# leotimus/recommender-tensorflow

Hardware: AMD Instinct MI355X
Metric: examples/sec DeepFM batch=65536 (full train step) (higher is better)
Workload: dtype f32 (MLP GEMM operands: fp16 hi+lo split, 3 products, fp32 accumulate)

## Files before the change

recommender-tensorflow_amd/csrc/gemm_pl.hip:

```cpp
#include "common.h"
#include "planes.h"
#include <algorithm>
#include <cstdlib>
#include <type_traits>

namespace {

typedef _Float16 f16x8 __attribute__((ext_vector_type(8)));
typedef float f32x16 __attribute__((ext_vector_type(16)));

constexpr int PL_THREADS = 512;
constexpr int PL_BK = 16;

enum { PL_FWD = 0, PL_DGRAD = 1, PL_TOP = 2 };

struct PlArgs {
  const char* A; int64_t bsa; const int32_t* a_exp;
  const char* B; int64_t bsb; const int32_t* b_exp;
  int M, N, K;
  int tiles_n;
  float* C; int64_t ldc;
  char* Cp; int64_t bsc; int32_t* c_exp;
  const float* bias; int relu; float keep_prob, keep_div, keep_rcp; uint64_t seed;
  const char* mask; int64_t bsm;
  uint32_t* mbits; int64_t mbld;
  float* amax_c;
  const mi_step_state_t* st;
  const float* top_w; const float* top_b;
  const float* top_lin; const float* top_lin_bias; const float* top_fm; const uint8_t* top_labels; float top_scale;
  float* top_dnn; float* top_logits; float* top_dlogit;
  float* top_part;
};

#ifdef MI_PL_STAMPS
__device__ long long g_pl_stamps[32 * 2 * 128 * 8];
#define PL_STAMP(slot) do { if (stamp_on && t < 128) g_pl_stamps[((stamp_wg * 2 + stamp_grp) * 128 + t) * 8 + (slot)] = clock64(); } while (0)
#define PL_MARK(row) do { if (stamp_on) g_pl_stamps[((stamp_wg * 2 + stamp_grp) * 128 + (row)) * 8 + 7] = clock64(); } while (0)
#else
#define PL_STAMP(slot) do {} while (0)
#define PL_MARK(row) do {} while (0)
#endif

template <int TN, int TM, int EPI, bool HOT = false>
__global__ __launch_bounds__(PL_THREADS, 2) void gemm_pl_k(const PlArgs a) {
  constexpr int PL_NBUF = TN == 1 ? 3 : 4;
  constexpr int BNt = 128 * TN, BMt = 64 * TM, ROWS = BNt + BMt;
  constexpr int LPS = ROWS * 4 / PL_THREADS;
  static_assert(ROWS * 4 % PL_THREADS == 0, "tile rows");
  constexpr int STAGE = ROWS * PL_ROWB;
  static_assert(PL_NBUF * STAGE <= 160 * 1024, "LDS");
  __shared__ __attribute__((aligned(1024))) char smem[PL_NBUF * STAGE];

  const int nb = gridDim.x, bid = blockIdx.x;
  const int qq = nb >> 3, rr = nb & 7, xcd = bid & 7, idx = bid >> 3;
  const int lid = (xcd < rr) ? xcd * (qq + 1) + idx : rr * (qq + 1) + (xcd - rr) * qq + idx;
  const int n0 = (lid % a.tiles_n) * BNt, m0 = (lid / a.tiles_n) * BMt;
  const int nk = a.K / PL_BK;

  const int t = threadIdx.x, lane = t & 63;
  const int wv = __builtin_amdgcn_readfirstlane(t >> 6);
  const int i = lane & 31, h = lane >> 5;
  const int wn = wv & 3, wm = wv >> 2;

  const char* src[LPS];
#pragma unroll
  for (int j = 0; j < LPS; ++j) {
    const int p = j * PL_THREADS + t;
    const int row = p >> 2, c = (p & 3) ^ ((row >> 2) & 3);
    if (j < TN) {
      const int n = min(n0 + row, a.N - 1);
      src[j] = a.A + static_cast<int64_t>(n) * PL_ROWB + c * 16;
    } else {
      const int m = min(m0 + row - BNt, a.M - 1);
      src[j] = a.B + static_cast<int64_t>(m) * PL_ROWB + c * 16;
    }
  }

  const int sw = (i >> 2) & 3;
  const int ch = (h ^ sw) * 16, cl = ((2 | h) ^ sw) * 16;
  const int offA = (wn * 32 * TN + i) * PL_ROWB;
  const int offB = (BNt + wm * 32 * TM + i) * PL_ROWB;

  f32x16 acc[TN][TM];
#pragma unroll
  for (int x = 0; x < TN; ++x)
#pragma unroll
    for (int y = 0; y < TM; ++y)
#pragma unroll
      for (int r = 0; r < 16; ++r) acc[x][y][r] = 0.f;

  auto issue_share = [&](int kt, int buf) {
#pragma unroll
    for (int j = 0; j < LPS; ++j)
      __builtin_amdgcn_global_load_lds((const __attribute__((address_space(1))) void*)(src[j] + kt * (j < TN ? a.bsa : a.bsb)),
                                       (__attribute__((address_space(3))) void*)(smem + buf * STAGE + (j * PL_THREADS + wv * 64) * 16),
                                       16, 0, 0);
  };
  f16x8 ah[TN], al[TN], bh[TM], bl[TM];
  auto read_frags = [&](int bufi) {
    const char* buf = smem + bufi * STAGE;
#pragma unroll
    for (int x = 0; x < TN; ++x) {
      ah[x] = *reinterpret_cast<const f16x8*>(buf + offA + x * 32 * PL_ROWB + ch);
      al[x] = *reinterpret_cast<const f16x8*>(buf + offA + x * 32 * PL_ROWB + cl);
    }
#pragma unroll
    for (int y = 0; y < TM; ++y) {
      bh[y] = *reinterpret_cast<const f16x8*>(buf + offB + y * 32 * PL_ROWB + ch);
      bl[y] = *reinterpret_cast<const f16x8*>(buf + offB + y * 32 * PL_ROWB + cl);
    }
  };
  constexpr bool DMA_IN_C = TN != 1;
  auto phase_c = [&](int t) {
    int fb = t - 1 + PL_NBUF;
    fb -= (fb / PL_NBUF) * PL_NBUF;
    const int kt = min(t - 1 + PL_NBUF, nk - 1);
    constexpr int NT = TN * TM, NM = 3 * NT, GAP = NM / (LPS + 1);
#pragma unroll
    for (int idx = 0; idx < NM; ++idx) {
      const int pr = idx / NT, x = (idx % NT) / TM, y = idx % TM;
      acc[x][y] = __builtin_amdgcn_mfma_f32_32x32x16_f16(pr == 0 ? al[x] : ah[x], pr == 1 ? bl[y] : bh[y], acc[x][y], 0, 0, 0);
      if (DMA_IN_C && (idx + 1) % GAP == 0 && (idx + 1) / GAP <= LPS) {
        const int j = (idx + 1) / GAP - 1;
        __builtin_amdgcn_sched_barrier(0);
        __builtin_amdgcn_global_load_lds((const __attribute__((address_space(1))) void*)(src[j] + kt * (j < TN ? a.bsa : a.bsb)),
                                         (__attribute__((address_space(3))) void*)(smem + fb * STAGE + (j * PL_THREADS + wv * 64) * 16),
                                         16, 0, 0);
        __builtin_amdgcn_sched_barrier(0);
      }
    }
  };
  auto phase_l = [&](int t) {
    if (!DMA_IN_C && t >= 1) {
      int fb = t - 1;
      fb -= (fb / PL_NBUF) * PL_NBUF;
      issue_share(min(t - 1 + PL_NBUF, nk - 1), fb);
    }
    int rb = t;
    rb -= (rb / PL_NBUF) * PL_NBUF;
    read_frags(rb);
  };
  const bool g1 = __builtin_amdgcn_readfirstlane(wm) != 0;

#ifdef MI_PL_STAMPS
  const int stamp_every = max(1, nb / 32);
  const bool stamp_on = lane == 0 && (wv == 0 || wv == 4) && lid % stamp_every == 0 && lid / stamp_every < 32;
  const int stamp_wg = lid / stamp_every, stamp_grp = wv >> 2;
#endif
  PL_MARK(0);
#pragma unroll
  for (int s = 0; s < PL_NBUF; ++s) issue_share(min(s, nk - 1), s);
  mi_wait_vmcnt<LPS*(PL_NBUF - 1)>();
  __builtin_amdgcn_s_barrier();
  if (g1) __builtin_amdgcn_s_barrier();
  PL_MARK(1);
#pragma unroll 1
  for (int t = 0; t < nk; ++t) {
    PL_STAMP(0);
    phase_l(t);
    PL_STAMP(1);
    asm volatile("s_waitcnt lgkmcnt(0)" ::: "memory");
    PL_STAMP(2);
    mi_wait_vmcnt<LPS*(DMA_IN_C ? PL_NBUF - 3 : PL_NBUF - 2)>();
    PL_STAMP(3);
    __builtin_amdgcn_sched_barrier(0);
    __builtin_amdgcn_s_barrier();
    __builtin_amdgcn_sched_barrier(0);
    PL_STAMP(4);
    __builtin_amdgcn_s_setprio(1);
    phase_c(t);
    __builtin_amdgcn_s_setprio(0);
    PL_STAMP(5);
    __builtin_amdgcn_sched_barrier(0);
    __builtin_amdgcn_s_barrier();
    __builtin_amdgcn_sched_barrier(0);
    PL_STAMP(6);
  }
  if (!g1) __builtin_amdgcn_s_barrier();
  PL_MARK(2);

  if constexpr (EPI == PL_TOP) {
    static_assert(TN == 1, "PL_TOP: one 128-column tile");
    mi_wait_vmcnt<0>();
    __syncthreads();
    float* e_fw = reinterpret_cast<float*>(smem);
    float* e_bias = e_fw + 128;
    float* e_w = e_bias + 128;
    float* e_part = e_w + 128;
    float* e_dw = e_part + 4 * BMt;
    float* e_sc = e_dw + 256;
    float* e_wmax = e_sc + 4;
    static_assert((128 * 3 + 4 * BMt + 256 + 4 + 8) * 4 <= 8192 && 8192 + 8 * 4096 <= PL_NBUF * STAGE, "PL_TOP LDS");
    char* wreg = smem + 8192 + wv * 4096;
    for (int n = t; n < 128; n += PL_THREADS) {
      const bool ok = n < a.N;
      e_fw[n] = ok ? pl_pow2(-a.a_exp[ok ? n : 0]) : 0.f;
      e_bias[n] = (a.bias && ok) ? a.bias[n] : 0.f;
      e_w[n] = ok ? a.top_w[n] : 0.f;
    }
    __syncthreads();
    const bool drop = a.keep_prob < 1.f;
    const uint32_t thresh16 = drop ? mi_drop_thresh16(a.keep_prob) : 0x10000u;
    const uint64_t seed = a.seed + (a.st ? a.st->seed_term : 0ull);
    const int nw = wn * 32;
    const uint32_t pair_base = static_cast<uint32_t>((nw + 4 * h) >> 1) * MI_DROP_PAIR_MUL;
    const float kd = a.keep_div, kr = a.keep_rcp;
    const float relu_floor = a.relu ? 0.f : -__builtin_inff();
    float wr[16];
#pragma unroll
    for (int g = 0; g < 4; ++g) {
// ... 133 lines not shown
      for (int q = 0; q < 4; ++q) {
        auto r1 = __builtin_amdgcn_permlane32_swap(ph[q], ph[q + 4], false, false);
        ph[q] = r1[0]; ph[q + 4] = r1[1];
        auto r2 = __builtin_amdgcn_permlane32_swap(pq[q], pq[q + 4], false, false);
        pq[q] = r2[0]; pq[q + 4] = r2[1];
      }
      char* d = wreg + (h * 32 + i) * 64;
      const int rot = (i >> 1) & 3;
      *reinterpret_cast<uint4*>(d + ((0 ^ rot) << 4)) = make_uint4(ph[0], ph[1], ph[4], ph[5]);
      *reinterpret_cast<uint4*>(d + ((1 ^ rot) << 4)) = make_uint4(ph[2], ph[3], ph[6], ph[7]);
      *reinterpret_cast<uint4*>(d + ((2 ^ rot) << 4)) = make_uint4(pq[0], pq[1], pq[4], pq[5]);
      *reinterpret_cast<uint4*>(d + ((3 ^ rot) << 4)) = make_uint4(pq[2], pq[3], pq[6], pq[7]);
      asm volatile("s_waitcnt lgkmcnt(0)" ::: "memory");
#pragma unroll
      for (int q = 0; q < 4; ++q) {
        const int off = q * 1024 + lane * 16;
        const int blk = off >> 11, row = (off >> 6) & 31, slot = (off >> 4) & 3;
        const uint4 v4 = *reinterpret_cast<const uint4*>(wreg + off);
        const int mm = m0 + wm * 32 * TM + y * 32 + row, ncol = nw + blk * 16;
        if (mm < a.M && ncol < a.N)
          *reinterpret_cast<uint4*>(a.Cp + (ncol >> 4) * a.bsc + static_cast<int64_t>(mm) * PL_ROWB + ((slot ^ ((row >> 1) & 3)) << 4)) = v4;
      }
      asm volatile("s_waitcnt lgkmcnt(0)" ::: "memory");
    }
    return;
  }

  mi_wait_vmcnt<0>();
  __syncthreads();
  float* e_fw = reinterpret_cast<float*>(smem);
  float* e_bias = e_fw + BNt;
  float* e_rmax = e_bias + BNt;
  float* e_wmax = e_rmax + 4 * BMt;
  constexpr int FS = TN * 128 + 16;
  constexpr int WREG = 32 * FS > TN * 4096 ? 32 * FS : TN * 4096;
  constexpr int WPR = BNt / 32;
  static_assert(8192 + 8 * WREG + BMt * WPR * 4 <= PL_NBUF * STAGE, "epilogue LDS");
  char* wreg = smem + 8192 + wv * WREG;
  uint32_t* e_bits = reinterpret_cast<uint32_t*>(smem + 8192 + 8 * WREG);
  for (int n = t; n < BNt; n += PL_THREADS) {
    const int gn = n0 + n;
    const bool ok = HOT || gn < a.N;
    e_fw[n] = ok ? pl_pow2(-a.a_exp[ok ? gn : 0]) : 0.f;
    e_bias[n] = (EPI == PL_FWD && a.bias && ok) ? a.bias[gn] : 0.f;
  }
  __syncthreads();

  const bool drop = EPI == PL_FWD && (HOT || a.keep_prob < 1.f);
  float* const Cf = HOT ? nullptr : a.C;
  const uint32_t thresh16 = drop ? mi_drop_thresh16(a.keep_prob) : 0x10000u;
  const uint64_t seed = a.seed + (a.st ? a.st->seed_term : 0ull);
  const int nw = wn * 32 * TN;
  const uint32_t pair_base = static_cast<uint32_t>((n0 + nw + 4 * h) >> 1) * MI_DROP_PAIR_MUL;
  const bool bitmask = EPI == PL_DGRAD && (HOT || a.mbits != nullptr);
  const bool masked = !HOT && EPI == PL_DGRAD && a.mask != nullptr && !bitmask;
  const bool divide = drop || masked || bitmask;
  const float kd = divide ? a.keep_div : 1.f, kr = divide ? a.keep_rcp : 1.f;
  const float relu_floor = a.relu ? 0.f : -__builtin_inff();
  float rmx[TM];
#pragma unroll
  for (int y = 0; y < TM; ++y) {
    const int m = m0 + wm * 32 * TM + y * 32 + i;
    const bool mok = HOT || m < a.M;
    const int mc = mok ? m : a.M - 1;
    const float fx = pl_pow2(-a.b_exp[mc]);
    float mx = 0.f;
    const uint32_t rowkey = drop ? mi_drop_rowkey(seed, static_cast<uint32_t>(m)) : 0u;
    auto col_of = [&](int gi) { return nw + (gi >> 2) * 32 + 8 * (gi & 3) + 4 * h; };
    float4 fw_n = *reinterpret_cast<const float4*>(e_fw + col_of(0));
    float4 b_n = make_float4(0.f, 0.f, 0.f, 0.f);
// ... 470 lines not shown
}

__global__ __launch_bounds__(256) void top_fold_k(const float* __restrict__ part, int nparts, int N, float* __restrict__ dW,
                                                  float* __restrict__ db, float* __restrict__ d_sum, float* __restrict__ loss) {
  __shared__ float red[16][17];
  const int c = threadIdx.x & 15, sl = threadIdx.x >> 4;
  const int k = blockIdx.x * 16 + c;
  float acc = 0.f;
  if (k < N + 2) {
#pragma unroll 8
    for (int q = sl; q < nparts; q += 16) acc += part[static_cast<int64_t>(q) * (N + 2) + k];
  }
  red[sl][c] = acc;
  __syncthreads();
  if (sl == 0 && k < N + 2) {
    float v = 0.f;
#pragma unroll
    for (int q = 0; q < 16; ++q) v += red[q][c];
    if (k < N) dW[k] = v;
    else if (k == N) { if (db) db[0] = v; if (d_sum) d_sum[0] = v; }
    else if (loss) loss[0] = v;
  }
}

template <int EPI>
int32_t launch_pl(PlArgs& a, hipStream_t st, const char* what) {
  int tn = a.N <= 128 ? 1 : (a.N <= 256 ? 2 : 4);
  if (a.N > 512) tn = 2;
  if (const int v = mi::env_int("MI_PL_TILE", 0)) {
    if ((v == 1 || v == 2 || v == 4) && (!a.Cp || a.N <= 128 * v)) tn = v;
  }
  int tm = tn == 4 ? 2 : 4;
  if (tm == 4 && static_cast<int64_t>((a.N + 128 * tn - 1) / (128 * tn)) * ((a.M + 255) / 256) < 256) tm = 2;
  const int bn = 128 * tn, bm = 64 * tm;
  a.tiles_n = (a.N + bn - 1) / bn;
  const int64_t blocks = static_cast<int64_t>(a.tiles_n) * ((a.M + bm - 1) / bm);
  if (blocks <= 0 || blocks > INT32_MAX) {
    mi::set_error("%s: bad grid", what);
    return MI_ERR_INVALID;
  }
  if (a.Cp && a.tiles_n != 1) {
    mi::set_error("%s: a planes result needs N <= 512 (one column tile holds the whole row)", what);
    return MI_ERR_UNSUPPORTED;
  }
  const dim3 g(static_cast<unsigned>(blocks)), b(PL_THREADS);
  const bool hot = a.Cp && !a.C && a.tiles_n == 1 && a.N == bn && a.M % bm == 0 && a.amax_c && a.bsc < (int64_t(1) << 31) &&
                   (EPI == PL_FWD ? (a.keep_prob < 1.f && a.mbits && a.mbld * 32 == a.N && a.bias)
                                  : (a.mbits && a.mbld * 32 == a.N));
  if (hot && tn == 1 && tm == 4) gemm_pl_k<1, 4, EPI, true><<<g, b, 0, st>>>(a);
  else if (hot && tn == 2 && tm == 4) gemm_pl_k<2, 4, EPI, true><<<g, b, 0, st>>>(a);
  else if (hot && tn == 4 && EPI == PL_DGRAD) gemm_pl_k<4, 2, PL_DGRAD, true><<<g, b, 0, st>>>(a);
  else if (tn == 1 && tm == 4) gemm_pl_k<1, 4, EPI><<<g, b, 0, st>>>(a);
  else if (tn == 1) gemm_pl_k<1, 2, EPI><<<g, b, 0, st>>>(a);
  else if (tn == 2 && tm == 4) gemm_pl_k<2, 4, EPI><<<g, b, 0, st>>>(a);
  else if (tn == 2) gemm_pl_k<2, 2, EPI><<<g, b, 0, st>>>(a);
  else gemm_pl_k<4, 2, EPI><<<g, b, 0, st>>>(a);
  MI_CHECK_LAUNCH(what);
  return MI_OK;
}

}

extern "C" {

size_t mi_planes_bytes(int64_t rows, int32_t K) { return static_cast<size_t>((K + 15) >> 4) * static_cast<size_t>(rows) * PL_ROWB; }

int32_t mi_split_rows(const float* X, int64_t ldx, int64_t rows, int32_t K, int32_t transpose, const mi_planes_t* out,
                      float* amax_out, mi_stream_t stream) {
  MI_REQUIRE(rows >= 0 && K > 0 && X, "split_rows: rows=%lld K=%d", (long long)rows, K);
  if (rows == 0) return MI_OK;
  MI_REQUIRE(mi::planes_ok(out, rows), "split_rows: output planes (16-byte aligned data, blk_stride >= 64 * rows and a multiple of 64, row_exp)");
  MI_REQUIRE(transpose ? ldx >= rows : ldx >= K, "split_rows: ldx=%lld", (long long)ldx);
  if (transpose) {
    const int64_t tb = mi::ceil_div(rows, 32);
    MI_REQUIRE(tb <= INT32_MAX, "split_rows: grid too large");
    split_t_k<<<dim3((unsigned)tb), dim3(256), 0, mi::as_stream(stream)>>>(X, ldx, rows, K, static_cast<char*>(out->data),
                                                                           out->blk_stride, out->row_exp, amax_out);
    MI_CHECK_LAUNCH("split_rows(transposed)");
    return MI_OK;
  }
  if ((K & 15) == 0 && (ldx & 3) == 0 && (reinterpret_cast<uintptr_t>(X) & 15u) == 0) {
    int lpr = 1;
    while (lpr < 64 && lpr < (K >> 4)) lpr <<= 1;
// ... 57 lines not shown
  MI_CHECK_LAUNCH("merge_rows");
  return MI_OK;
}

int32_t mi_dense_fwd_planes(const mi_planes_t* X, const mi_planes_t* Wt, const float* bias, float* Y, int64_t ldy,
                            const mi_planes_t* Yp, int64_t M, int32_t N, int32_t K, int32_t relu, float keep_prob,
                            uint64_t seed, float* amax_out, uint32_t* mask_bits_out, int64_t mask_ld, mi_stream_t stream) {
  MI_REQUIRE(M >= 0 && M <= INT32_MAX && N > 0 && K > 0, "dense_fwd_planes: M=%lld N=%d K=%d", (long long)M, N, K);
  MI_REQUIRE(!mask_bits_out || mask_ld >= (N + 31) / 32, "dense_fwd_planes: mask_ld=%lld < ceil(N / 32)", (long long)mask_ld);
  if (M == 0) return MI_OK;
  MI_REQUIRE((K & 15) == 0 && (N & 15) == 0, "dense_fwd_planes: N=%d and K=%d must be multiples of 16 (use mi_dense_fwd)", N, K);
  MI_REQUIRE(mi::planes_ok(X, M) && mi::planes_ok(Wt, N), "dense_fwd_planes: operand planes");
  MI_REQUIRE(Y || Yp, "dense_fwd_planes: no output");
  MI_REQUIRE(!Y || (ldy >= N && (ldy & 3) == 0 && mi::aligned16(Y)), "dense_fwd_planes: Y leading dimension / alignment");
  MI_REQUIRE(!Yp || mi::planes_ok(Yp, M), "dense_fwd_planes: output planes");
  MI_REQUIRE(keep_prob > 0.f && keep_prob <= 1.f, "dense_fwd_planes: keep_prob=%f", keep_prob);
  PlArgs a{};
  a.A = static_cast<const char*>(Wt->data); a.bsa = Wt->blk_stride; a.a_exp = Wt->row_exp;
  a.B = static_cast<const char*>(X->data); a.bsb = X->blk_stride; a.b_exp = X->row_exp;
  a.M = (int)M; a.N = N; a.K = K;
  a.C = Y; a.ldc = ldy;
  if (Yp) { a.Cp = static_cast<char*>(Yp->data); a.bsc = Yp->blk_stride; a.c_exp = Yp->row_exp; }
  a.bias = bias; a.relu = relu; a.keep_prob = keep_prob; a.keep_div = keep_prob; a.keep_rcp = 1.0f / keep_prob; a.seed = seed; a.st = mi::step_state();
  a.amax_c = amax_out;
  a.mbits = mask_bits_out; a.mbld = mask_ld;
  return launch_pl<PL_FWD>(a, mi::as_stream(stream), "dense_fwd_planes");
}

int32_t mi_dense_bwd_data_planes(const mi_planes_t* dY, const mi_planes_t* W, const mi_planes_t* Xact, float* dX,
                                 int64_t lddx, const mi_planes_t* dXp, int64_t M, int32_t N, int32_t K, float keep_prob,
                                 float* amax_out, const uint32_t* mask_bits, int64_t mask_ld, mi_stream_t stream) {
  MI_REQUIRE(M >= 0 && M <= INT32_MAX && N > 0 && K > 0, "dense_bwd_data_planes: M=%lld N=%d K=%d", (long long)M, N, K);
  if (M == 0) return MI_OK;
  MI_REQUIRE((K & 15) == 0 && (N & 15) == 0, "dense_bwd_data_planes: N=%d and K=%d must be multiples of 16", N, K);
  MI_REQUIRE(mi::planes_ok(dY, M) && mi::planes_ok(W, K), "dense_bwd_data_planes: operand planes");
  MI_REQUIRE(!Xact || mi::planes_ok(Xact, M), "dense_bwd_data_planes: activation planes");
  MI_REQUIRE(!mask_bits || mask_ld >= (K + 31) / 32, "dense_bwd_data_planes: mask_ld=%lld < ceil(K / 32)", (long long)mask_ld);
  MI_REQUIRE(dX || dXp, "dense_bwd_data_planes: no output");
  MI_REQUIRE(!dX || (lddx >= K && (lddx & 3) == 0 && mi::aligned16(dX)), "dense_bwd_data_planes: dX leading dimension / alignment");
  MI_REQUIRE(!dXp || mi::planes_ok(dXp, M), "dense_bwd_data_planes: output planes");
  MI_REQUIRE(keep_prob > 0.f && keep_prob <= 1.f, "dense_bwd_data_planes: keep_prob=%f", keep_prob);
  PlArgs a{};
  a.A = static_cast<const char*>(W->data); a.bsa = W->blk_stride; a.a_exp = W->row_exp;
  a.B = static_cast<const char*>(dY->data); a.bsb = dY->blk_stride; a.b_exp = dY->row_exp;
  a.M = (int)M; a.N = K; a.K = N;
  a.C = dX; a.ldc = lddx;
  if (dXp) { a.Cp = static_cast<char*>(dXp->data); a.bsc = dXp->blk_stride; a.c_exp = dXp->row_exp; }
  a.keep_prob = keep_prob; a.keep_div = (Xact || mask_bits) ? keep_prob : 1.f; a.keep_rcp = 1.0f / a.keep_div;
  if (Xact) { a.mask = static_cast<const char*>(Xact->data); a.bsm = Xact->blk_stride; }
  a.mbits = const_cast<uint32_t*>(mask_bits); a.mbld = mask_ld;
  a.amax_c = amax_out;
  return launch_pl<PL_DGRAD>(a, mi::as_stream(stream), "dense_bwd_data_planes");
}


size_t mi_hidden_logits_head_fused_workspace_bytes(int64_t M, int32_t N) {
  if (M <= 0 || N <= 0) return 256;
  return static_cast<size_t>(mi::ceil_div(M, 128)) * (N + 2) * sizeof(float) + 256;
}

int32_t mi_hidden_logits_head_fused(const mi_planes_t* X, const mi_planes_t* Wt, const float* bias, int64_t M, int32_t N, int32_t K,
                                    int32_t relu, float keep_prob, uint64_t seed, const float* w, const float* b, const float* lin,
                                    const float* lin_bias, const float* fm, const uint8_t* labels, float loss_scale, float* dnn,
                                    float* logits, float* loss_out, float* d_logit, float* d_logit_sum, float* dW, float* db,
                                    const mi_planes_t* dXp, float* amax_out, void* workspace, size_t workspace_bytes,
                                    mi_stream_t stream) {
  MI_REQUIRE(M > 0 && M <= INT32_MAX && N == 128 && K > 0 && (K & 15) == 0,
// ... 86 lines not shown
```

recommender-tensorflow_amd/csrc/sort.hip:

```cpp
#include "common.h"

namespace {

constexpr int kBlock = 256;
constexpr int kItems = 16;
constexpr int kTile = kBlock * kItems;
constexpr int kMaxBits = 9;
constexpr int kMaxBins = 1 << kMaxBits;
constexpr int kMaxPasses = 4;
constexpr int kFusedMaxBits = 10;
constexpr int kFusedMaxBins = 1 << kFusedMaxBits;
constexpr int kFusedMaxTps = 256;

__global__ __launch_bounds__(256) void zero_i32_k(int32_t* __restrict__ p, int64_t n) {
  for (int64_t i = static_cast<int64_t>(blockIdx.x) * 256 + threadIdx.x; i < n; i += static_cast<int64_t>(gridDim.x) * 256) p[i] = 0;
}
inline void zero_i32(int32_t* p, int64_t n, hipStream_t st) {
  const int64_t b = (n + 255) / 256;
  zero_i32_k<<<dim3(static_cast<unsigned>(b < 64 ? b : 64)), dim3(256), 0, st>>>(p, n);
}

__global__ __launch_bounds__(kBlock) void hist_k(const int32_t* __restrict__ keys, int64_t n, int shift,
                                                 int nbins, int tps, int32_t* __restrict__ hist,
                                                 int32_t* __restrict__ bin_total) {
// ... 221 lines not shown
  const int64_t base = static_cast<int64_t>(blockIdx.x) * kTile;
  int run = tile_base[blockIdx.x];
  for (int r = 0; r < kItems; ++r) {
    const int64_t i = base + r * kBlock + t;
    const bool valid = i < n;
    int32_t key = 0;
    bool head = false;
    if (valid) {
      key = keys[i];
      head = is_head(keys, i, seg_len);
      sorted_entry[i] = vals[i];
    }
    const unsigned long long hb = __ballot(head);
    __syncthreads();
    if (lane == 0) wc[w] = __popcll(hb);
    __syncthreads();
    int idx = run + __popcll(hb & lt_mask);
    for (int ww = 0; ww < w; ++ww) idx += wc[ww];
    if (head) {
      uniq_rows[idx] = seg_len > 0 ? static_cast<int32_t>(field_off[i / seg_len] + key) : key;
      seg_start[idx] = static_cast<int32_t>(i);
    }
    if (slot_of_entry && valid) slot_of_entry[vals[i]] = head ? idx : idx - 1;
    run += wc[0] + wc[1] + wc[2] + wc[3];
  }
  if (blockIdx.x == 0 && t == 0) {
    const int32_t U = total[0];
    num_uniq[0] = U;
    seg_start[U] = static_cast<int32_t>(n);
  }
}

constexpr int kFieldsMax = 64;
__global__ __launch_bounds__(kBlock) void ids_field_major_k(const int32_t* __restrict__ ids, int64_t B, int F,
                                                            int32_t* __restrict__ out) {
  __shared__ int32_t tile[64][kFieldsMax + 1];
  const int64_t b0 = static_cast<int64_t>(blockIdx.x) * 64;
  const int nb = static_cast<int>(min(static_cast<int64_t>(64), B - b0));
  for (int i = threadIdx.x; i < nb * F; i += kBlock) tile[i / F][i % F] = ids[b0 * F + i];
  __syncthreads();
  for (int i = threadIdx.x; i < F * 64; i += kBlock) {
    const int f = i >> 6, bl = i & 63;
    if (bl < nb) out[static_cast<int64_t>(f) * B + b0 + bl] = tile[bl][f];
  }
}


__device__ __forceinline__ void st_agent(int32_t* p, int32_t v) { __hip_atomic_store(p, v, __ATOMIC_RELAXED, __HIP_MEMORY_SCOPE_AGENT); }
__device__ __forceinline__ int32_t ld_agent(const int32_t* p) { return __hip_atomic_load(p, __ATOMIC_RELAXED, __HIP_MEMORY_SCOPE_AGENT); }
constexpr int kSpinMax = 1 << 22;

template <int MAXBINS>
__global__ __launch_bounds__(kBlock) void pass_fused_k(const int32_t* __restrict__ keys_in, const int32_t* __restrict__ vals_in,
                                                       const int32_t* __restrict__ ids, int64_t B, int F, int shift, int nbits,
                                                       int tps, int32_t* __restrict__ thist, int32_t* __restrict__ ready,
                                                       int32_t* __restrict__ err, int32_t* __restrict__ keys_out,
                                                       int32_t* __restrict__ vals_out, int nap) {
  __shared__ int32_t running[4][MAXBINS];
  __shared__ int32_t offsT[MAXBINS];
  __shared__ int32_t totS[MAXBINS];
  __shared__ int32_t wsum[4];
  const int t = threadIdx.x, w = t >> 6, lane = t & 63;
  const int nbins = 1 << nbits;
  const int seg = blockIdx.x / tps, tis = blockIdx.x - seg * tps;
  for (int b = t; b < 4 * MAXBINS; b += kBlock) (&running[0][0])[b] = 0;
  __syncthreads();
  const int64_t base = static_cast<int64_t>(blockIdx.x) * kTile + w * (64 * kItems);
  int32_t key[kItems], val[kItems];
#pragma unroll
  for (int r = 0; r < kItems; ++r) {
    const int64_t i = base + r * 64 + lane;
    if (ids) {
      const int64_t e = (i - static_cast<int64_t>(seg) * B) * F + seg;
      key[r] = ids[e];
      val[r] = static_cast<int32_t>(e);
    } else {
// ... 385 lines not shown
  if (tps <= kFusedMaxTps && !beside && mi::env_int("MI_SORT_FUSED", 1) != 0) {
    const int fbits = mi::env_int("MI_SORT_BITS", 7) < kFusedMaxBits ? mi::env_int("MI_SORT_BITS", 7) : kFusedMaxBits;
    const int fpasses = (bits + fbits - 1) / fbits;
    const int fnb = (bits + fpasses - 1) / fpasses;
    MI_REQUIRE(fpasses <= kMaxPasses, "sort_unique_fields: %d passes", fpasses);
    int32_t* sync = reinterpret_cast<int32_t*>(ws + L.sync);
    int32_t* ready = sync;
    int32_t* hcf = sync + static_cast<int64_t>(kMaxPasses) * F;
    int32_t* err = hcf + ntiles;
    zero_i32(sync, L.sync_words, st);
    MI_CHECK_LAUNCH("sort_unique_fields(zero)");
    const int32_t* kin = nullptr;
    const int32_t* vin = nullptr;
    const int nap = mi::env_int("MI_SORT_NAP", 1);
    for (int p = 0; p < fpasses; ++p) {
      int32_t* kout = kbuf[p & 1];
      int32_t* vout = vbuf[p & 1];
      if (fnb > 9)
        pass_fused_k<kFusedMaxBins><<<dim3(ntiles), dim3(kBlock), 0, st>>>(kin, vin, p == 0 ? ids : nullptr, B, F, fnb * p, fnb, tps, hist,
                                                                          ready + static_cast<int64_t>(p) * F, err, kout, vout, nap);
      else
        pass_fused_k<kMaxBins><<<dim3(ntiles), dim3(kBlock), 0, st>>>(kin, vin, p == 0 ? ids : nullptr, B, F, fnb * p, fnb, tps, hist,
                                                                      ready + static_cast<int64_t>(p) * F, err, kout, vout, nap);
      MI_CHECK_LAUNCH("sort_unique_fields(pass)");
      kin = kout;
      vin = vout;
    }
    compact_fused_k<<<dim3(ntiles), dim3(kBlock), 0, st>>>(kin, vin, n, hcf, err, sorted_entry, uniq_rows, seg_start, num_uniq, B, field_off);
    MI_CHECK_LAUNCH("sort_unique_fields(compact)");
    return MI_OK;
  }
  zero_i32(bin_total, static_cast<int64_t>(kMaxPasses) * F * kMaxBins, st);
  MI_CHECK_LAUNCH("sort_unique_fields(zero)");
  ids_field_major_k<<<dim3((unsigned)mi::ceil_div(B, 64)), dim3(kBlock), 0, st>>>(ids, B, F, kbuf[1]);
  MI_CHECK_LAUNCH("sort_unique_fields(transpose)");
  const int32_t* kin = kbuf[1];
  const int32_t* vin = nullptr;
  for (int p = 0; p < passes; ++p) {
    int32_t* kout = kbuf[p & 1];
    int32_t* vout = vbuf[p & 1];
    int32_t* bt = bin_total + static_cast<int64_t>(p) * F * kMaxBins;
    hist_k<<<dim3(ntiles), dim3(kBlock), 0, st>>>(kin, n, nbits * p, nbins, tps, hist, bt);
    MI_CHECK_LAUNCH("sort_unique_fields(hist)");
    bin_scan_k<<<dim3(F * nbins), dim3(kBlock), 0, st>>>(hist, tps, nbins, bt, B);
    MI_CHECK_LAUNCH("sort_unique_fields(scan)");
    scatter_k<<<dim3(ntiles), dim3(kBlock), 0, st>>>(kin, vin, n, nbits * p, nbits, tps, hist, kout, vout, p == 0 ? B : 0, F);
    MI_CHECK_LAUNCH("sort_unique_fields(scatter)");
    kin = kout;
    vin = vout;
  }
  head_count_k<<<dim3(ntiles), dim3(kBlock), 0, st>>>(kin, n, heads, B);
  MI_CHECK_LAUNCH("sort_unique_fields(heads)");
  scan_small_k<<<dim3(1), dim3(kScanSmallBlock), 0, st>>>(heads, ntiles, total);
  MI_CHECK_LAUNCH("sort_unique_fields(scan heads)");
  compact_k<<<dim3(ntiles), dim3(kBlock), 0, st>>>(kin, vin, n, heads, total, sorted_entry, uniq_rows, seg_start, num_uniq, B, field_off);
  MI_CHECK_LAUNCH("sort_unique_fields(compact)");
  return MI_OK;
}

}

namespace {

__global__ __launch_bounds__(kBlock) void shard_keys_k(const int32_t* __restrict__ rows, int64_t n, int world,
                                                       int64_t entries_per_chunk, int64_t rows_per_rank, int self_rank,
                                                       int32_t* __restrict__ keys) {
  const int64_t i = static_cast<int64_t>(blockIdx.x) * kBlock + threadIdx.x;
  if (i >= n) return;
  const int32_t r = rows[i];
  const int64_t chunk = entries_per_chunk > 0 ? i / entries_per_chunk : 0;
  int o = r % world;
  if (self_rank >= 0) o = o == self_rank ? world - 1 : (o > self_rank ? o - 1 : o);
  keys[i] = static_cast<int32_t>((chunk * world + o) * rows_per_rank + r / world);
}

__global__ __launch_bounds__(kBlock) void route_requests_k(const int32_t* __restrict__ uniq_keys,
                                                           const int32_t* __restrict__ num_uniq, int64_t rows_per_rank,
                                                           int32_t* __restrict__ send_rows, int32_t* __restrict__ counts) {
  const int64_t u = static_cast<int64_t>(blockIdx.x) * kBlock + threadIdx.x;
  const int64_t U = *num_uniq;
  if (u >= U) return;
  const int64_t key = uniq_keys[u];
  const int64_t grp = key / rows_per_rank;
  send_rows[u] = static_cast<int32_t>(key - grp * rows_per_rank);
  if (u + 1 == U) {
    atomicAdd(counts + grp, static_cast<int32_t>(U));
  } else {
    const int64_t gn = static_cast<int64_t>(uniq_keys[u + 1]) / rows_per_rank;
// ... 84 lines not shown
```

Baseline: 23.79 million.

## Use 2x2 tile with higher occupancy for hot 256-wide GEMMs, skip dead MFMAs

For the hot path (N=256, one column tile, planar output), the kernel now uses a TN=2,TM=2 tile with three LDS buffers and launch bounds allowing four workgroups per CU instead of two, trading per-block reuse for occupancy. For non-hot TN=2 kernels it computes per-wave how many 32-column fragments are live and dispatches a specialised K loop that skips MFMAs on columns beyond N. The LDS size now covers the epilogue requirement explicitly, and dgrad input validation is relaxed to allow K multiples of 4 for fp32 outputs. Risks: lower operand reuse with smaller tiles, register pressure under the tighter launch bound, and larger code from the per-LIVE specialisations.

Measured after the change: 23.73 million. No clear change (-0.2%).

```diff
diff --git a/recommender-tensorflow_amd/csrc/gemm_pl.hip b/recommender-tensorflow_amd/csrc/gemm_pl.hip
--- a/recommender-tensorflow_amd/csrc/gemm_pl.hip
+++ b/recommender-tensorflow_amd/csrc/gemm_pl.hip
@@ -42,14 +42,21 @@
 #endif
 
 template <int TN, int TM, int EPI, bool HOT = false>
-__global__ __launch_bounds__(PL_THREADS, 2) void gemm_pl_k(const PlArgs a) {
-  constexpr int PL_NBUF = TN == 1 ? 3 : 4;
+__global__ __launch_bounds__(PL_THREADS, (HOT && TN == 2 && TM == 2) ? 4 : 2) void gemm_pl_k(const PlArgs a) {
+  constexpr bool PAIR = HOT && TN == 2 && TM == 2;
+  constexpr int PL_NBUF = (TN == 1 || PAIR) ? 3 : 4;
   constexpr int BNt = 128 * TN, BMt = 64 * TM, ROWS = BNt + BMt;
   constexpr int LPS = ROWS * 4 / PL_THREADS;
   static_assert(ROWS * 4 % PL_THREADS == 0, "tile rows");
   constexpr int STAGE = ROWS * PL_ROWB;
-  static_assert(PL_NBUF * STAGE <= 160 * 1024, "LDS");
-  __shared__ __attribute__((aligned(1024))) char smem[PL_NBUF * STAGE];
+  constexpr int FS = TN * 128 + 16;
+  constexpr int WREG = (!PAIR && 32 * FS > TN * 4096) ? 32 * FS : TN * 4096;
+  constexpr int WPR = BNt / 32;
+  constexpr int EPI_LDS = 8192 + 8 * WREG + BMt * WPR * 4;
+  constexpr int SMEM = PL_NBUF * STAGE > EPI_LDS ? PL_NBUF * STAGE : EPI_LDS;
+  static_assert(SMEM <= 160 * 1024 && (!(TN == 1 || PAIR) || SMEM <= 80 * 1024), "LDS");
+  static_assert(EPI == PL_TOP || PAIR || EPI_LDS <= PL_NBUF * STAGE, "epilogue LDS");
+  __shared__ __attribute__((aligned(1024))) char smem[SMEM];
 
   const int nb = gridDim.x, bid = blockIdx.x;
   const int qq = nb >> 3, rr = nb & 7, xcd = bid & 7, idx = bid >> 3;
@@ -110,8 +117,11 @@
       bl[y] = *reinterpret_cast<const f16x8*>(buf + offB + y * 32 * PL_ROWB + cl);
     }
   };
+  constexpr bool RAGGED = TN == 2 && !HOT;
+  const int live = RAGGED ? __builtin_amdgcn_readfirstlane(min(max((a.N - n0 - wn * 32 * TN + 31) >> 5, 0), TN)) : TN;
   constexpr bool DMA_IN_C = TN != 1;
-  auto phase_c = [&](int t) {
+  auto phase_c = [&](int t, auto live_c) {
+    constexpr int LIVE = decltype(live_c)::value;
     int fb = t - 1 + PL_NBUF;
     fb -= (fb / PL_NBUF) * PL_NBUF;
     const int kt = min(t - 1 + PL_NBUF, nk - 1);
@@ -119,7 +129,8 @@
 #pragma unroll
     for (int idx = 0; idx < NM; ++idx) {
       const int pr = idx / NT, x = (idx % NT) / TM, y = idx % TM;
-      acc[x][y] = __builtin_amdgcn_mfma_f32_32x32x16_f16(pr == 0 ? al[x] : ah[x], pr == 1 ? bl[y] : bh[y], acc[x][y], 0, 0, 0);
+      if (x < LIVE)
+        acc[x][y] = __builtin_amdgcn_mfma_f32_32x32x16_f16(pr == 0 ? al[x] : ah[x], pr == 1 ? bl[y] : bh[y], acc[x][y], 0, 0, 0);
       if (DMA_IN_C && (idx + 1) % GAP == 0 && (idx + 1) / GAP <= LPS) {
         const int j = (idx + 1) / GAP - 1;
         __builtin_amdgcn_sched_barrier(0);
@@ -154,28 +165,37 @@
   __builtin_amdgcn_s_barrier();
   if (g1) __builtin_amdgcn_s_barrier();
   PL_MARK(1);
+  auto k_loop = [&](auto live_c) {
 #pragma unroll 1
-  for (int t = 0; t < nk; ++t) {
-    PL_STAMP(0);
-    phase_l(t);
-    PL_STAMP(1);
-    asm volatile("s_waitcnt lgkmcnt(0)" ::: "memory");
-    PL_STAMP(2);
-    mi_wait_vmcnt<LPS*(DMA_IN_C ? PL_NBUF - 3 : PL_NBUF - 2)>();
-    PL_STAMP(3);
-    __builtin_amdgcn_sched_barrier(0);
-    __builtin_amdgcn_s_barrier();
-    __builtin_amdgcn_sched_barrier(0);
-    PL_STAMP(4);
-    __builtin_amdgcn_s_setprio(1);
-    phase_c(t);
-    __builtin_amdgcn_s_setprio(0);
-    PL_STAMP(5);
-    __builtin_amdgcn_sched_barrier(0);
-    __builtin_amdgcn_s_barrier();
-    __builtin_amdgcn_sched_barrier(0);
-    PL_STAMP(6);
-  }
+    for (int t = 0; t < nk; ++t) {
+      PL_STAMP(0);
+      phase_l(t);
+      PL_STAMP(1);
+      asm volatile("s_waitcnt lgkmcnt(0)" ::: "memory");
+      PL_STAMP(2);
+      mi_wait_vmcnt<LPS*(DMA_IN_C ? PL_NBUF - 3 : PL_NBUF - 2)>();
+      PL_STAMP(3);
+      __builtin_amdgcn_sched_barrier(0);
+      __builtin_amdgcn_s_barrier();
+      __builtin_amdgcn_sched_barrier(0);
+      PL_STAMP(4);
+      __builtin_amdgcn_s_setprio(1);
+      phase_c(t, live_c);
+      __builtin_amdgcn_s_setprio(0);
+      PL_STAMP(5);
+      __builtin_amdgcn_sched_barrier(0);
+      __builtin_amdgcn_s_barrier();
+      __builtin_amdgcn_sched_barrier(0);
+      PL_STAMP(6);
+    }
+  };
+  auto k_loop_for = [&](auto self, auto live_c) {
+    constexpr int LIVE = decltype(live_c)::value;
+    if (live == LIVE) k_loop(live_c);
+    else if constexpr (LIVE > 0) self(self, std::integral_constant<int, LIVE - 1>{});
+  };
+  if constexpr (RAGGED) k_loop_for(k_loop_for, std::integral_constant<int, TN>{});
+  else k_loop(std::integral_constant<int, TN>{});
   if (!g1) __builtin_amdgcn_s_barrier();
   PL_MARK(2);
 
@@ -375,10 +395,6 @@
   float* e_bias = e_fw + BNt;
   float* e_rmax = e_bias + BNt;
   float* e_wmax = e_rmax + 4 * BMt;
-  constexpr int FS = TN * 128 + 16;
-  constexpr int WREG = 32 * FS > TN * 4096 ? 32 * FS : TN * 4096;
-  constexpr int WPR = BNt / 32;
-  static_assert(8192 + 8 * WREG + BMt * WPR * 4 <= PL_NBUF * STAGE, "epilogue LDS");
   char* wreg = smem + 8192 + wv * WREG;
   uint32_t* e_bits = reinterpret_cast<uint32_t*>(smem + 8192 + 8 * WREG);
   for (int n = t; n < BNt; n += PL_THREADS) {
@@ -915,6 +931,10 @@
   }
   int tm = tn == 4 ? 2 : 4;
   if (tm == 4 && static_cast<int64_t>((a.N + 128 * tn - 1) / (128 * tn)) * ((a.M + 255) / 256) < 256) tm = 2;
+  const bool hot_opts = a.Cp && !a.C && a.amax_c && a.bsc < (int64_t(1) << 31) &&
+                        (EPI == PL_FWD ? (a.keep_prob < 1.f && a.mbits && a.mbld * 32 == a.N && a.bias)
+                                       : (a.mbits && a.mbld * 32 == a.N));
+  if (hot_opts && tn == 2 && a.N == 256 && a.M % 128 == 0) tm = 2;
   const int bn = 128 * tn, bm = 64 * tm;
   a.tiles_n = (a.N + bn - 1) / bn;
   const int64_t blocks = static_cast<int64_t>(a.tiles_n) * ((a.M + bm - 1) / bm);
@@ -927,11 +947,9 @@
     return MI_ERR_UNSUPPORTED;
   }
   const dim3 g(static_cast<unsigned>(blocks)), b(PL_THREADS);
-  const bool hot = a.Cp && !a.C && a.tiles_n == 1 && a.N == bn && a.M % bm == 0 && a.amax_c && a.bsc < (int64_t(1) << 31) &&
-                   (EPI == PL_FWD ? (a.keep_prob < 1.f && a.mbits && a.mbld * 32 == a.N && a.bias)
-                                  : (a.mbits && a.mbld * 32 == a.N));
+  const bool hot = hot_opts && a.tiles_n == 1 && a.N == bn && a.M % bm == 0;
   if (hot && tn == 1 && tm == 4) gemm_pl_k<1, 4, EPI, true><<<g, b, 0, st>>>(a);
-  else if (hot && tn == 2 && tm == 4) gemm_pl_k<2, 4, EPI, true><<<g, b, 0, st>>>(a);
+  else if (hot && tn == 2 && tm == 2) gemm_pl_k<2, 2, EPI, true><<<g, b, 0, st>>>(a);
   else if (hot && tn == 4 && EPI == PL_DGRAD) gemm_pl_k<4, 2, PL_DGRAD, true><<<g, b, 0, st>>>(a);
   else if (tn == 1 && tm == 4) gemm_pl_k<1, 4, EPI><<<g, b, 0, st>>>(a);
   else if (tn == 1) gemm_pl_k<1, 2, EPI><<<g, b, 0, st>>>(a);
@@ -1055,7 +1073,8 @@
                                  float* amax_out, const uint32_t* mask_bits, int64_t mask_ld, mi_stream_t stream) {
   MI_REQUIRE(M >= 0 && M <= INT32_MAX && N > 0 && K > 0, "dense_bwd_data_planes: M=%lld N=%d K=%d", (long long)M, N, K);
   if (M == 0) return MI_OK;
-  MI_REQUIRE((K & 15) == 0 && (N & 15) == 0, "dense_bwd_data_planes: N=%d and K=%d must be multiples of 16", N, K);
+  MI_REQUIRE((N & 15) == 0 && (K & 3) == 0 && ((K & 15) == 0 || (!dXp && !Xact)),
+             "dense_bwd_data_planes: N=%d and K=%d must be multiples of 16 (K: of 4 for an fp32 result without activation planes)", N, K);
   MI_REQUIRE(mi::planes_ok(dY, M) && mi::planes_ok(W, K), "dense_bwd_data_planes: operand planes");
   MI_REQUIRE(!Xact || mi::planes_ok(Xact, M), "dense_bwd_data_planes: activation planes");
   MI_REQUIRE(!mask_bits || mask_ld >= (K + 31) / 32, "dense_bwd_data_planes: mask_ld=%lld < ceil(K / 32)", (long long)mask_ld);
```

## Restructure per-field radix sort: fuse transpose, pack pairs, self-compute offsets, fold head scan

Applied to the files above, without the earlier changes.

Drops the separate field-major transpose kernel by having the first histogram and scatter passes read ids directly with strided indexing. Intermediate passes store keys and values as packed int2 pairs, and the scatter stages a tile in shared memory so global writes become runs. When the histogram is small, each scatter block computes its own global offsets, which removes the bin_scan launch. The head-count scan is folded into the compact kernel. Together these cut kernel launches and memory traffic in the non-fused sort path, at the cost of redundant per-block prefix work and heavier shared-memory use.

Measured after the change: 24.93 million before, 25.18 million after, median of 6. 1.01x the previous value.

```diff
diff --git a/recommender-tensorflow_amd/csrc/sort.hip b/recommender-tensorflow_amd/csrc/sort.hip
--- a/recommender-tensorflow_amd/csrc/sort.hip
+++ b/recommender-tensorflow_amd/csrc/sort.hip
@@ -277,16 +277,189 @@
 }
 
 constexpr int kFieldsMax = 64;
-__global__ __launch_bounds__(kBlock) void ids_field_major_k(const int32_t* __restrict__ ids, int64_t B, int F,
-                                                            int32_t* __restrict__ out) {
-  __shared__ int32_t tile[64][kFieldsMax + 1];
-  const int64_t b0 = static_cast<int64_t>(blockIdx.x) * 64;
-  const int nb = static_cast<int>(min(static_cast<int64_t>(64), B - b0));
-  for (int i = threadIdx.x; i < nb * F; i += kBlock) tile[i / F][i % F] = ids[b0 * F + i];
-  __syncthreads();
-  for (int i = threadIdx.x; i < F * 64; i += kBlock) {
-    const int f = i >> 6, bl = i & 63;
-    if (bl < nb) out[static_cast<int64_t>(f) * B + b0 + bl] = tile[bl][f];
+
+__device__ __forceinline__ int32_t fields_key(const int2* __restrict__ pairs_in, const int32_t* __restrict__ ids, int64_t i,
+                                              int seg, int64_t B, int F) {
+  return ids ? ids[(i - static_cast<int64_t>(seg) * B) * F + seg] : pairs_in[i].x;
+}
+
+__global__ __launch_bounds__(kBlock) void hist_fields_k(const int2* __restrict__ pairs_in, const int32_t* __restrict__ ids, int64_t B,
+                                                        int F, int shift, int nbins, int tps, int32_t* __restrict__ hist,
+                                                        int32_t* __restrict__ bin_total) {
+  __shared__ unsigned int h[kMaxBins];
+  for (int b = threadIdx.x; b < nbins; b += kBlock) h[b] = 0;
+  __syncthreads();
+  const int seg = blockIdx.x / tps, tis = blockIdx.x - seg * tps;
+  const int64_t base = static_cast<int64_t>(blockIdx.x) * kTile;
+  const unsigned int mask = nbins - 1;
+#pragma unroll
+  for (int r = 0; r < kItems; ++r)
+    atomicAdd(&h[(static_cast<uint32_t>(fields_key(pairs_in, ids, base + r * kBlock + threadIdx.x, seg, B, F)) >> shift) & mask], 1u);
+  __syncthreads();
+  for (int b = threadIdx.x; b < nbins; b += kBlock) {
+    const unsigned int c = h[b];
+    hist[(static_cast<int64_t>(seg) * nbins + b) * tps + tis] = static_cast<int32_t>(c);
+    if (c) atomicAdd(&bin_total[seg * nbins + b], static_cast<int32_t>(c));
+  }
+}
+
+constexpr int kSelfOffsMaxInts = 4096;
+
+template <bool IDS>
+__global__ __launch_bounds__(kBlock) void scatter_runs_k(const int2* __restrict__ pairs_in, const int32_t* __restrict__ ids, int64_t B,
+                                                         int F, int shift, int nbits, int tps, const int32_t* __restrict__ hist,
+                                                         const int32_t* __restrict__ bin_total, int self_offs,
+                                                         int2* __restrict__ pairs_out, int32_t* __restrict__ keys_out,
+                                                         int32_t* __restrict__ vals_out) {
+  __shared__ int2 staged[kTile];
+  __shared__ int32_t running[4][kMaxBins];
+  int32_t* before = reinterpret_cast<int32_t*>(staged);
+  int32_t* tstart = before + kMaxBins;
+  int32_t (*cnt)[kMaxBins] = reinterpret_cast<int32_t (*)[kMaxBins]>(tstart + kMaxBins);
+  int32_t (*wsum)[4] = reinterpret_cast<int32_t (*)[4]>(cnt + 4);
+  const int t = threadIdx.x, w = t >> 6, lane = t & 63;
+  const int nbins = 1 << nbits;
+  const int seg = blockIdx.x / tps, tis = blockIdx.x - seg * tps;
+  for (int b = t; b < 4 * kMaxBins; b += kBlock) (&cnt[0][0])[b] = 0;
+  for (int b = t; b < nbins; b += kBlock) before[b] = 0;
+  __syncthreads();
+  const int64_t base = static_cast<int64_t>(blockIdx.x) * kTile + w * (64 * kItems);
+  const int32_t e0 = static_cast<int32_t>((base - static_cast<int64_t>(seg) * B + lane) * F + seg);
+  int32_t key[kItems], val[IDS ? 1 : kItems];
+#pragma unroll
+  for (int r = 0; r < kItems; ++r) {
+    if (IDS) {
+      key[r] = ids[e0 + r * 64 * F];
+    } else {
+      const int2 kv = pairs_in[base + r * 64 + lane];
+      key[r] = kv.x;
+      val[r] = kv.y;
+    }
+    atomicAdd(&cnt[w][(static_cast<uint32_t>(key[r]) >> shift) & (nbins - 1)], 1);
+  }
+  const int32_t* fh = hist + static_cast<int64_t>(seg) * nbins * tps;
+  if (self_offs)
+    for (int i = t; i < nbins * tps; i += kBlock) {
+      const int b = i / tps;
+      if (i - b * tps < tis) atomicAdd(&before[b], fh[i]);
+    }
+  __syncthreads();
+  const int per = nbins > kBlock ? nbins / kBlock : 1;
+  int32_t delta[kMaxBins / kBlock];
+  {
+    int32_t tc[kMaxBins / kBlock], tot[kMaxBins / kBlock];
+    int own_c = 0, own_t = 0;
+#pragma unroll
+    for (int j = 0; j < kMaxBins / kBlock; ++j) {
+      const int b = t * per + j;
+      tc[j] = tot[j] = 0;
+      if (j < per && b < nbins) {
+        tc[j] = cnt[0][b] + cnt[1][b] + cnt[2][b] + cnt[3][b];
+        if (self_offs) tot[j] = bin_total[seg * nbins + b];
+      }
+      own_c += tc[j];
+      own_t += tot[j];
+    }
+    const int incl_c = wave_incl_scan(own_c, lane), incl_t = wave_incl_scan(own_t, lane);
+    if (lane == 63) { wsum[0][w] = incl_c; wsum[1][w] = incl_t; }
+    __syncthreads();
+    int pre_c = incl_c - own_c, pre_t = incl_t - own_t + static_cast<int>(static_cast<int64_t>(seg) * B);
+    for (int ww = 0; ww < w; ++ww) { pre_c += wsum[0][ww]; pre_t += wsum[1][ww]; }
+#pragma unroll
+    for (int j = 0; j < kMaxBins / kBlock; ++j) {
+      const int b = t * per + j;
+      delta[j] = 0;
+      if (j < per && b < nbins) {
+        const int32_t gofs = self_offs ? pre_t + before[b] : fh[static_cast<int64_t>(b) * tps + tis];
+        delta[j] = gofs - pre_c;
+        tstart[b] = pre_c;
+        pre_c += tc[j];
+        pre_t += tot[j];
+      }
+    }
+  }
+  __syncthreads();
+  for (int b = lane; b < nbins; b += 64) {
+    int32_t f = tstart[b];
+    for (int ww = 0; ww < w; ++ww) f += cnt[ww][b];
+    running[w][b] = f;
+  }
+  __syncthreads();
+  const unsigned long long lt_mask = (lane == 0) ? 0ull : (~0ull >> (64 - lane));
+  int32_t* run = running[w];
+#pragma unroll
+  for (int r = 0; r < kItems; ++r) {
+    asm volatile("" : "+v"(key[r]));
+    const unsigned int d = (static_cast<uint32_t>(key[r]) >> shift) & (nbins - 1);
+    unsigned long long peers = ~0ull;
+    for (int b = 0; b < nbits; ++b) {
+      const unsigned long long m = __ballot((d >> b) & 1u);
+      peers &= ((d >> b) & 1u) ? m : ~m;
+    }
+    const int rank = __popcll(peers & lt_mask);
+    const int32_t dst = lds_ld(run + d) + rank;
+    __builtin_amdgcn_wave_barrier();
+    if (rank == 0) lds_st(run + d, dst + __popcll(peers));
+    staged[dst] = make_int2(key[r], IDS ? e0 + r * 64 * F : val[r]);
+    __builtin_amdgcn_wave_barrier();
+  }
+  __syncthreads();
+#pragma unroll
+  for (int j = 0; j < kMaxBins / kBlock; ++j)
+    if (j < per && t * per + j < nbins) running[0][t * per + j] = delta[j];
+  __syncthreads();
+#pragma unroll
+  for (int r = 0; r < kItems; ++r) {
+    const int s = r * kBlock + t;
+    const int2 kv = staged[s];
+    const int32_t dst = running[0][(static_cast<uint32_t>(kv.x) >> shift) & (nbins - 1)] + s;
+    if (keys_out) {
+      keys_out[dst] = kv.x;
+      vals_out[dst] = kv.y;
+    } else {
+      pairs_out[dst] = kv;
+    }
+  }
+}
+
+constexpr int kFoldHeadsMaxTiles = 4096;
+__global__ __launch_bounds__(kBlock) void compact_fields_k(const int32_t* __restrict__ keys, const int32_t* __restrict__ vals, int64_t n,
+                                                           const int32_t* __restrict__ tile_heads, int32_t* __restrict__ sorted_entry,
+                                                           int32_t* __restrict__ uniq_rows, int32_t* __restrict__ seg_start,
+                                                           int32_t* __restrict__ num_uniq, int64_t seg_len,
+                                                           const int64_t* __restrict__ field_off) {
+  __shared__ int32_t red[4];
+  __shared__ int32_t wc[4];
+  const int t = threadIdx.x, w = t >> 6, lane = t & 63;
+  const unsigned long long lt_mask = (lane == 0) ? 0ull : (~0ull >> (64 - lane));
+  const int64_t base = static_cast<int64_t>(blockIdx.x) * kTile;
+  int part = 0;
+  for (int j = t; j < static_cast<int>(blockIdx.x); j += kBlock) part += tile_heads[j];
+#pragma unroll
+  for (int off = 32; off > 0; off >>= 1) part += __shfl_xor(part, off, 64);
+  if (lane == 0) red[w] = part;
+  __syncthreads();
+  int run = red[0] + red[1] + red[2] + red[3];
+  for (int r = 0; r < kItems; ++r) {
+    const int64_t i = base + r * kBlock + t;
+    const int32_t key = keys[i];
+    const bool head = is_head(keys, i, seg_len);
+    sorted_entry[i] = vals[i];
+    const unsigned long long hb = __ballot(head);
+    __syncthreads();
+    if (lane == 0) wc[w] = __popcll(hb);
+    __syncthreads();
+    if (head) {
+      int idx = run + __popcll(hb & lt_mask);
+      for (int ww = 0; ww < w; ++ww) idx += wc[ww];
+      uniq_rows[idx] = static_cast<int32_t>(field_off[i / seg_len] + key);
+      seg_start[idx] = static_cast<int32_t>(i);
+    }
+    run += wc[0] + wc[1] + wc[2] + wc[3];
+  }
+  if (blockIdx.x == gridDim.x - 1 && t == 0) {
+    num_uniq[0] = run;
+    seg_start[run] = static_cast<int32_t>(n);
   }
 }
 
@@ -738,28 +911,41 @@
   }
   zero_i32(bin_total, static_cast<int64_t>(kMaxPasses) * F * kMaxBins, st);
   MI_CHECK_LAUNCH("sort_unique_fields(zero)");
-  ids_field_major_k<<<dim3((unsigned)mi::ceil_div(B, 64)), dim3(kBlock), 0, st>>>(ids, B, F, kbuf[1]);
-  MI_CHECK_LAUNCH("sort_unique_fields(transpose)");
-  const int32_t* kin = kbuf[1];
-  const int32_t* vin = nullptr;
+  static_assert(sizeof(int2) == 8, "pair buffers");
+  int2* pbuf[2] = {reinterpret_cast<int2*>(kbuf[0]), reinterpret_cast<int2*>(vbuf[0])};
+  const bool self_offs = static_cast<int64_t>(nbins) * tps <= kSelfOffsMaxInts;
+  const int2* pin = nullptr;
+  int32_t* kout = nullptr;
+  int32_t* vout = nullptr;
   for (int p = 0; p < passes; ++p) {
-    int32_t* kout = kbuf[p & 1];
-    int32_t* vout = vbuf[p & 1];
+    const bool last = p == passes - 1;
     int32_t* bt = bin_total + static_cast<int64_t>(p) * F * kMaxBins;
-    hist_k<<<dim3(ntiles), dim3(kBlock), 0, st>>>(kin, n, nbits * p, nbins, tps, hist, bt);
+    hist_fields_k<<<dim3(ntiles), dim3(kBlock), 0, st>>>(pin, p == 0 ? ids : nullptr, B, F, nbits * p, nbins, tps, hist, bt);
     MI_CHECK_LAUNCH("sort_unique_fields(hist)");
-    bin_scan_k<<<dim3(F * nbins), dim3(kBlock), 0, st>>>(hist, tps, nbins, bt, B);
-    MI_CHECK_LAUNCH("sort_unique_fields(scan)");
-    scatter_k<<<dim3(ntiles), dim3(kBlock), 0, st>>>(kin, vin, n, nbits * p, nbits, tps, hist, kout, vout, p == 0 ? B : 0, F);
+    if (!self_offs) {
+      bin_scan_k<<<dim3(F * nbins), dim3(kBlock), 0, st>>>(hist, tps, nbins, bt, B);
+      MI_CHECK_LAUNCH("sort_unique_fields(scan)");
+    }
+    kout = last ? (p & 1 ? vbuf[0] : kbuf[0]) : nullptr;
+    vout = last ? (p & 1 ? vbuf[1] : kbuf[1]) : nullptr;
+    if (p == 0)
+      scatter_runs_k<true><<<dim3(ntiles), dim3(kBlock), 0, st>>>(nullptr, ids, B, F, 0, nbits, tps, hist, bt, self_offs ? 1 : 0,
+                                                                  last ? nullptr : pbuf[0], kout, vout);
+    else
+      scatter_runs_k<false><<<dim3(ntiles), dim3(kBlock), 0, st>>>(pin, nullptr, B, F, nbits * p, nbits, tps, hist, bt, self_offs ? 1 : 0,
+                                                                   last ? nullptr : pbuf[p & 1], kout, vout);
     MI_CHECK_LAUNCH("sort_unique_fields(scatter)");
-    kin = kout;
-    vin = vout;
-  }
-  head_count_k<<<dim3(ntiles), dim3(kBlock), 0, st>>>(kin, n, heads, B);
+    pin = pbuf[p & 1];
+  }
+  head_count_k<<<dim3(ntiles), dim3(kBlock), 0, st>>>(kout, n, heads, B);
   MI_CHECK_LAUNCH("sort_unique_fields(heads)");
-  scan_small_k<<<dim3(1), dim3(kScanSmallBlock), 0, st>>>(heads, ntiles, total);
-  MI_CHECK_LAUNCH("sort_unique_fields(scan heads)");
-  compact_k<<<dim3(ntiles), dim3(kBlock), 0, st>>>(kin, vin, n, heads, total, sorted_entry, uniq_rows, seg_start, num_uniq, B, field_off);
+  if (ntiles <= kFoldHeadsMaxTiles) {
+    compact_fields_k<<<dim3(ntiles), dim3(kBlock), 0, st>>>(kout, vout, n, heads, sorted_entry, uniq_rows, seg_start, num_uniq, B, field_off);
+  } else {
+    scan_small_k<<<dim3(1), dim3(kScanSmallBlock), 0, st>>>(heads, ntiles, total);
+    MI_CHECK_LAUNCH("sort_unique_fields(scan heads)");
+    compact_k<<<dim3(ntiles), dim3(kBlock), 0, st>>>(kout, vout, n, heads, total, sorted_entry, uniq_rows, seg_start, num_uniq, B, field_off);
+  }
   MI_CHECK_LAUNCH("sort_unique_fields(compact)");
   return MI_OK;
 }
```
